# aticejiang/MLAgg-UNet

Hardware: AMD Instinct MI355X
Metric: images/sec (train step) MLAgg-UNet-2D 256x256 bs10 (higher is better)
Workload: dtype f32; 1 GPU; nnUNetTrainer_MLAgg_2D_dt_MS train step, AbdomenMRI-shaped 256x256x1, 14 classes, attention variant B (BASELINE.json configs[1]); batch_per_gpu=10, global_batch=10, parallelism=dp1, launch=eager, miopen=tuned find-db (mlagg-unet_amd/miopen_db), library_gemm=TunableOp table (mlagg-unet_amd/gemm_db), tuning off

## Files before the change

include/mlagg_hip.h:

```cpp
#ifndef MLAGG_HIP_H
#define MLAGG_HIP_H

#include <stddef.h>

#ifdef __cplusplus
extern "C" {
#endif

#define MLAGG_E_UNSUPPORTED (-1)
#define MLAGG_E_NULLPTR     (-2)
#define MLAGG_E_WORKSPACE   (-3)

#define MLAGG_DTYPE_F32  0
#define MLAGG_DTYPE_BF16 1
#define MLAGG_DTYPE_F16  2
#define MLAGG_DTYPE_BF16X3 3

const char *mlagg_version(void);
const char *mlagg_error_string(int code);

int mlagg_profile_kernel_count(void);
const char *mlagg_profile_kernel_name(int id);
int mlagg_profile_select(int id);
int mlagg_profile_collect(double *ms, int *counts);
// ... 55 lines not shown
                              float *dbias, float *workspace, int batch, int H, int W, int C, void *stream);
int mlagg_dwconv3x3_bwd(const float *x, int x_stride, const float *w, const float *dy, int dy_stride,
                        const float *pre, float *dx, int dx_stride, float *dw, float *dbias, float *workspace,
                        int batch, int H, int W, int C, int silu, void *stream);

int mlagg_linear_fwd(const float *x, int x_stride, const float *w, const float *bias, float *y, int y_stride,
                     int M, int N, int K, void *stream);
int mlagg_linear_dgrad(const float *dy, int dy_stride, const float *w, float *dx, int dx_stride, int M, int O, int I,
                       void *stream);
int mlagg_linear_lp_fwd(const float *x, int x_stride, const float *w, const float *bias, float *y, int y_stride,
                        int M, int N, int K, int dtype, void *stream);
int mlagg_linear_lp_dgrad(const float *dy, int dy_stride, const float *w, float *dx, int dx_stride, int M, int O, int I,
                          int dtype, void *stream);
size_t mlagg_linear_wgrad_workspace_floats(int M, int O, int I);
int mlagg_linear_wgrad(const float *dy, int dy_stride, const float *x, int x_stride, float *dW, float *db,
                       float *workspace, int M, int O, int I, void *stream);
int mlagg_linear_wgrad_x3(const float *dy, int dy_stride, const float *x, int x_stride, float *dW, float *db, float *workspace,
                          int M, int O, int I, void *stream);

int mlagg_flash_attn_fwd(const void *q, const void *k, const void *v, void *out, float *lse, int B, int N, int P, int nh,
                         int head_dim, float softmax_scale, int dtype, void *stream);
size_t mlagg_flash_attn_bwd_workspace_floats(int B, int N, int P, int nh, int head_dim);
int mlagg_flash_attn_bwd(const void *q, const void *k, const void *v, const void *out, const void *dout, const float *lse,
                         void *dq, float *workspace, int B, int N, int P, int nh, int head_dim, float softmax_scale,
                         int dtype, void *stream);

int mlagg_layernorm_supported(int C);
int mlagg_layernorm_fwd(const float *x, int x_stride, const float *gamma, const float *beta, float *y,
                        float *stats, int rows, int C, float eps, void *stream);
size_t mlagg_layernorm_bwd_workspace_floats(int rows, int C);
int mlagg_layernorm_bwd(const float *x, int x_stride, const float *dy, int dy_stride, const float *gamma,
                        const float *stats, float *dx, float *dgamma, float *dbeta, float *workspace,
                        int rows, int C, void *stream);
int mlagg_residual_layernorm_fwd(const float *skip, const float *branch, const float *scale, const float *gamma, const float *beta,
                                 float *xsum, float *y, float *stats, int rows, int rows_per_sample, int C, float eps, void *stream);
int mlagg_residual_layernorm_bwd(const float *xsum, const float *dy, int dy_stride, const float *dres, const float *scale,
                                 const float *gamma, const float *stats, float *dskip, float *dbranch, float *dgamma, float *dbeta,
                                 float *workspace, int rows, int rows_per_sample, int C, void *stream);

int mlagg_dwconv3d_fwd(const float *x, int x_stride, const float *w, const float *bias, float *y, int y_stride,
                       float *pre, int batch, int D, int H, int W, int C, int silu, void *stream);
size_t mlagg_dwconv3d_bwd_workspace_floats(int batch, int D, int H, int W, int C);
int mlagg_dwconv3d_bwd(const float *x, int x_stride, const float *w, const float *dy, int dy_stride, const float *pre,
                       float *dx, int dx_stride, float *dw, float *dbias, float *workspace, int batch, int D, int H,
                       int W, int C, int silu, void *stream);

int mlagg_dwconv3x3_nchw_fwd(const float *x, const float *w, const float *bias, float *y, int B, int C, int H, int W,
                             int stride, void *stream);
size_t mlagg_dwconv3x3_nchw_bwd_workspace_floats(int B, int C, int H, int W, int stride);
int mlagg_dwconv3x3_nchw_bwd(const float *x, const float *w, const float *dy, float *dx, float *dw, float *dbias,
                             float *workspace, int B, int C, int H, int W, int stride, void *stream);
int mlagg_dwconv3x3_nchw_bwd_res(const float *x, const float *w, const float *dy, const float *dres, float *dx, float *dw, float *dbias,
                                 float *workspace, int B, int C, int H, int W, int stride, void *stream);

int mlagg_cross_scan(const float *tok, int tok_stride, int blk_stride, float *seq, int B, int nscale,
                     const int *H, const int *W, int CB, int nblk, void *stream);
int mlagg_cross_merge(const float *seq, float *tok, int tok_stride, int blk_stride, int B, int nscale,
                      const int *H, const int *W, int CB, int nblk, void *stream);

int mlagg_conv1x1_supported(int O, int I, long P);
int mlagg_conv1x1_fwd(const float *x, long x_batch, const float *w, const float *bias, float *y, long y_batch, int B, int O, int I,
                      long P, void *stream);
size_t mlagg_conv1x1_wgrad_workspace_floats(int B, int O, int I, long P);
int mlagg_conv1x1_wgrad(const float *dy, long dy_batch, const float *x, long x_batch, float *dW, float *workspace, int B, int O,
                        int I, long P, void *stream);
int mlagg_conv1x1_fwd_lp(const float *x, long x_batch, const float *w, const float *bias, float *y, long y_batch, int B, int O, int I,
                         long P, int dtype, void *stream);
int mlagg_conv1x1_wgrad_lp(const float *dy, long dy_batch, const float *x, long x_batch, float *dW, float *workspace, int B, int O,
                           int I, long P, int dtype, void *stream);
int mlagg_conv1x1_fwd_ragged(const float *x, long x_batch, const float *w, const float *bias, float *y, long y_batch, int B, int O, int I,
                             int I_valid, long P, int dtype, void *stream);
int mlagg_conv1x1_fwd_acc(const float *x, long x_batch, const float *w, const float *bias, float *y, long y_batch, int B, int O, int I,
                          int I_valid, long P, int dtype, int accumulate, void *stream);
int mlagg_conv1x1_fwd_tile(int O);
int mlagg_conv1x1_wgrad_tile(int O, int I);

int mlagg_conv3x3_supported(int O, int I, int H, int W);
size_t mlagg_conv3x3_workspace_bytes(int O, int I);
int mlagg_conv3x3_fwd(const float *x, long x_batch, const float *w, int transposed, const float *bias, float *y, long y_batch,
                      void *workspace, int B, int O, int I, int H, int W, void *stream);
int mlagg_conv3x3x3_supported(int O, int I, int D, int H, int W);
size_t mlagg_conv3x3x3_workspace_bytes(int O, int I);
int mlagg_conv3x3x3_fwd(const float *x, long x_batch, const float *w, int transposed, const float *bias, float *y, long y_batch,
                        void *workspace, int B, int O, int I, int D, int H, int W, void *stream);
int mlagg_conv3x3_wgrad_supported(int O, int I, int H, int W);
int mlagg_conv3x3x3_wgrad_supported(int O, int I, int D, int H, int W);
size_t mlagg_conv3x3x3_wgrad_workspace_floats(int B, int O, int I, int D, int H, int W);
int mlagg_conv3x3x3_wgrad(const float *dy, long dy_batch, const float *x, long x_batch, float *dW, float *workspace, int B, int O,
                          int I, int D, int H, int W, void *stream);
size_t mlagg_conv3x3_wgrad_workspace_floats(int B, int O, int I, int H, int W);
int mlagg_conv3x3_wgrad(const float *dy, long dy_batch, const float *x, long x_batch, float *dW, float *workspace, int B, int O,
                        int I, int H, int W, void *stream);
int mlagg_conv3x3_fwd_lp(const float *x, long x_batch, const float *w, int transposed, const float *bias, float *y, long y_batch,
                         void *workspace, int B, int O, int I, int H, int W, int dtype, void *stream);
int mlagg_conv3x3_wgrad_lp(const float *dy, long dy_batch, const float *x, long x_batch, float *dW, float *workspace, int B, int O,
                           int I, int H, int W, int dtype, void *stream);
int mlagg_conv3x3_fwd_tile(int O, int D, int H, int W);
int mlagg_conv3x3_wgrad_form(int O, int I, int D, int dtype);

int mlagg_conv3x3_s2t_supported(int O, int I, int H, int W);
size_t mlagg_conv3x3_s2t_workspace_bytes(int O, int I);
int mlagg_conv3x3_s2t_fwd(const float *x, long x_batch, const float *w, float *y, long y_batch, void *workspace, int B, int O, int I,
                          int H, int W, int dtype, void *stream);
int mlagg_conv3x3_s2_dgrad(const float *dy, long dy_batch, long dy_chan_stride, long dy_row_stride, const float *w, float *dx,
                           long dx_batch, void *workspace, int B, int O, int I, int H, int W, int dtype, void *stream);
size_t mlagg_conv3x3_s2t_wgrad_workspace_floats(int B, int O, int I, int H, int W);
// ... 242 lines not shown
```

mlagg-unet_amd/csrc/api.hip:

```cpp
#include <hip/hip_runtime.h>

#include <mutex>
#include <vector>

#include "mlagg_hip.h"
#include "prof.h"

namespace mlagg_prof {

int g_selected = -1;

namespace {
struct Rec {
    int id;
    hipEvent_t start, stop;
};
std::mutex g_mu;
std::vector<Rec> g_recs;
size_t g_used = 0;
const char *const kNames[K_COUNT] = {
    "selscan_fwd_kernel<false>", "selscan_chunk_prefix", "selscan_fwd_kernel<true>", "selscan_bwd_local_kernel",
    "selscan_bwd_group_kernel", "selscan_reduce_partials", "local_attn_fwd_kernel", "local_attn_bwd_a_kernel",
    "local_attn_bwd_b_kernel", "pooled_attn_fwd_kernel", "pooled_attn_bwd1_kernel",
    "pooled_attn_bwd2_kernel", "dwconv_tiled_kernel<fwd>", "dwconv_tiled_kernel<dgrad>", "dwconv_bwd_weight_kernel", "linear weight gradient (K5w: linear_wgrad_kernel / linear_wgrad_x3_kernel + reduce)", "layernorm_fwd_kernel",
    "layernorm_bwd_kernel", "dwconv_nchw_fwd_kernel", "dwconv_nchw_bwd (data+weight+reduce)",
    "cross_scan_kernel<false>", "cross_scan_kernel<true>", "gate_fwd_kernel", "gate_bwd_kernel",
    "linear forward + data gradient (K5: linear_x3_kernel on weight images; MLAGG_K5_V2=0: linear_lp_kernel<true, MODE> / linear_mfma_kernel<true>)", "linear data gradient (K5: linear_mfma_kernel<false> / linear_lp_kernel<false, MODE>)", "row_scale_kernel", "dice_ce_stats_kernel", "dice_ce_grad_kernel", "transpose_tile_kernel", "bias gradient (plane_sum / column_sum)", "plane_norm_fwd_kernel", "plane_norm_bwd_kernel", "adamw (sumsq + update)", "flash_fwd_kernel", "flash_bwd (dq + dk/dv)", "channel_epilogue (bias + residual + GELU)",
    "sel1_fwd_kernel<2, false>", "sel1_fwd_kernel<2, true>", "sel1_bwd_local_kernel<2>", "sel1_bwd_kernel<2>",
    "sel1_fwd_kernel<R != 2, false>", "sel1_fwd_kernel<R != 2, true>", "sel1_bwd_local_kernel<R != 2>", "sel1_bwd_kernel<R != 2>",
    "sel1_prefix_kernel", "sel1 reductions (step partials + per-chunk rows)",
    "volume_pad_kernel (+ guard fill)", "conv_wgrad_taps_kernel", "conv_wgrad_reduce_kernel", "conv_taps_kernel (forward / data gradient)",
    "gelu_pool (forward + backward)", "conv1x1 (forward / data gradient / weight gradient)",
    "conv3x3 (forward / data gradient / weight gradient, incl. weight image and reduce)",
    "tok_fwd_kernel<false>", "tok_fwd_kernel<true>", "tok_bwd_local_kernel", "tok_bwd_group_kernel",
    "sw_gather_kernel", "sw_fold_kernel", "sw_finalize_kernel", "resample_linear_kernel", "export_kernel",
    "pp_box_kernel", "pp_stats_kernel (+ final)", "pp_normalize_kernel", "pp_minmax_kernel", "pp_cubic_kernel", "pp_gather_kernel",
    "cc_local_kernel", "cc_merge_kernel", "cc_compress_kernel", "cc_size_kernel", "cc_max_kernel", "cc_write_kernel",
    "sf_stats_kernel (+ init)", "sf_codes_kernel", "sf_zpass_kernel", "sf_ypass_kernel", "sf_xpass_kernel", "sf_sum_kernel",
    "aug3d_resample_kernel", "pt_seg_crop_kernel", "pt_seg_resize_kernel", "pt_rank_count_kernel (+ scan)", "pt_rank_select_kernel",
    "cl_local_kernel", "cl_merge_kernel", "cl_compress_kernel", "cl_flag_kernel", "cl_scan (count + offsets + apply)", "cl_rewrite_kernel",
    "cl_overlap_kernel", "cl_match_kernel", "ens_mean_kernel", "label_confusion_kernel", "dice_bce_stats_kernel", "dice_bce_grad_kernel",
    "aug3d_planar_kernel", "sw_gather_onehot_kernel"};
}

void record(int id, hipStream_t st, bool begin)
{
    std::lock_guard<std::mutex> lk(g_mu);
    if (begin) {
        if (g_used == g_recs.size()) {
            Rec r{id, nullptr, nullptr};
            if (hipEventCreate(&r.start) != hipSuccess || hipEventCreate(&r.stop) != hipSuccess) return;
            g_recs.push_back(r);
        }
        g_recs[g_used].id = id;
        (void)hipEventRecord(g_recs[g_used].start, st);
        ++g_used;
    } else if (g_used > 0) {
        (void)hipEventRecord(g_recs[g_used - 1].stop, st);
    }
}

}

extern "C" const char *mlagg_version(void) { return "mlagg_hip 0.1 (gfx950)"; }

extern "C" const char *mlagg_error_string(int code)
{
    switch (code) {
    case 0: return "success";
    case MLAGG_E_UNSUPPORTED: return "unsupported shape for the gfx950 kernels";
    case MLAGG_E_NULLPTR: return "required pointer argument is NULL";
    case MLAGG_E_WORKSPACE: return "workspace too small";
    default: return code > 0 ? hipGetErrorString(static_cast<hipError_t>(code)) : "unknown mlagg error";
    }
}

extern "C" int mlagg_profile_kernel_count(void) { return mlagg_prof::K_COUNT; }

extern "C" const char *mlagg_profile_kernel_name(int id)
{
    return (id >= 0 && id < mlagg_prof::K_COUNT) ? mlagg_prof::kNames[id] : "?";
}

extern "C" int mlagg_profile_select(int id)
{
    if (id < -2 || id >= mlagg_prof::K_COUNT) return MLAGG_E_UNSUPPORTED;
    mlagg_prof::g_selected = id;
    return 0;
}

extern "C" int mlagg_profile_collect(double *ms, int *counts)
{
    using namespace mlagg_prof;
    if (!ms || !counts) return MLAGG_E_NULLPTR;
    std::lock_guard<std::mutex> lk(g_mu);
// ... 12 lines not shown
```

mlagg-unet_amd/csrc/prof.h:

```cpp
#pragma once
#include <hip/hip_runtime.h>

namespace mlagg_prof {

enum KernelId {
    K_SELSCAN_FWD_LOCAL = 0, K_SELSCAN_PREFIX, K_SELSCAN_FWD_FINAL, K_SELSCAN_BWD_LOCAL, K_SELSCAN_BWD,
    K_SELSCAN_REDUCE, K_LOCAL_FWD, K_LOCAL_BWD_A, K_LOCAL_BWD_B, K_POOLED_FWD,
    K_POOLED_BWD1, K_POOLED_BWD2, K_DWCONV_FWD, K_DWCONV_BWD_DATA, K_DWCONV_BWD_WEIGHT, K_LINEAR_WGRAD, K_LAYERNORM_FWD, K_LAYERNORM_BWD, K_DWCONV_NCHW_FWD, K_DWCONV_NCHW_BWD, K_CROSS_SCAN, K_CROSS_MERGE, K_GATE_FWD, K_GATE_BWD, K_LINEAR_FWD, K_LINEAR_DGRAD, K_ROW_SCALE, K_LOSS_STATS, K_LOSS_GRAD, K_TRANSPOSE, K_BIAS_GRAD, K_PLANE_NORM_FWD, K_PLANE_NORM_BWD, K_ADAMW, K_FLASH_FWD, K_FLASH_BWD, K_CHANNEL_EPI,
    K_SEL1_FWD_LOCAL_R2, K_SEL1_FWD_FINAL_R2, K_SEL1_BWD_LOCAL_R2, K_SEL1_BWD_R2, K_SEL1_FWD_LOCAL, K_SEL1_FWD_FINAL, K_SEL1_BWD_LOCAL,
    K_SEL1_BWD, K_SEL1_PREFIX, K_SEL1_REDUCE, K_CONV_PAD, K_CONV_WGRAD, K_CONV_WGRAD_REDUCE, K_CONV_TAPS, K_GELU_POOL, K_CONV1X1, K_CONV3X3, K_TOK_FWD_LOCAL, K_TOK_FWD_FINAL, K_TOK_BWD_LOCAL, K_TOK_BWD_GROUP, K_SW_GATHER, K_SW_FOLD, K_SW_FINALIZE, K_RESAMPLE_LINEAR, K_EXPORT_SEG, K_PP_BOX, K_PP_STATS, K_PP_NORMALIZE, K_PP_MINMAX, K_PP_CUBIC, K_PP_GATHER, K_CC_LOCAL, K_CC_MERGE, K_CC_COMPRESS, K_CC_SIZE, K_CC_MAX, K_CC_WRITE, K_SF_STATS, K_SF_CODES, K_SF_ZPASS, K_SF_YPASS, K_SF_XPASS, K_SF_SUM, K_AUG3D_RESAMPLE, K_PT_SEG_CROP, K_PT_SEG_RESIZE, K_PT_RANK_COUNTS, K_PT_RANK_SELECT,
    K_CL_LOCAL, K_CL_MERGE, K_CL_COMPRESS, K_CL_FLAG, K_CL_SCAN, K_CL_REWRITE, K_CL_OVERLAP, K_CL_MATCH,
    K_ENS_MEAN, K_LABEL_CONFUSION, K_REGION_LOSS_STATS, K_REGION_LOSS_GRAD, K_AUG3D_PLANAR, K_SW_GATHER_ONEHOT, K_COUNT
};

extern int g_selected;
void record(int id, hipStream_t st, bool begin);

struct Scope {
    int id;
    hipStream_t st;
    bool on;
    Scope(int id_, hipStream_t st_) : id(id_), st(st_), on(g_selected == -2 || g_selected == id_)
    {
        if (on) record(id, st, true);
    }
    ~Scope()
    {
        if (on) record(id, st, false);
    }
};

}

#define MLAGG_TIMED(id, st) mlagg_prof::Scope mlagg_prof_scope_##id(mlagg_prof::id, st)
```

mlagg-unet_amd/model.py:

```python
import math
from typing import Sequence

import torch
import torch.nn as nn
import torch.nn.functional as F

from . import ops

LAMBDA_INIT = 0.8


class _DropPathPool:

    active = None

    def __init__(self):
        self.order, self.keep, self.masks, self.pos, self.recording = [], None, None, 0, False
        self.injected, self.forced = None, False

    def inject(self, factors):
        self.injected = factors

    def begin(self, batch, device):
        if self.injected is not None:
# ... 95 lines not shown
        y = self.raw(x)
        if y.dtype == torch.float32:
            return ops.channel_epilogue(y, self.bias, res if res is None or res.dtype == torch.float32 else res.float(), act)
        if y.numel() // (y.shape[0] * y.shape[1]) % 4:
            return ops.channel_epilogue(y.float(), self.bias, None if res is None else res.float(), act)
        return ops.channel_epilogue_lp(y, self.bias, res, act, dtype or torch.float32)

    def _device_forward(self, x):
        y = self.raw(x)
        if y.dtype == torch.float32:
            return y if self.bias is None else ops.channel_bias(y, self.bias)
        if y.numel() // (y.shape[0] * y.shape[1]) % 4:
            y = y.float()
            return y if self.bias is None else ops.channel_bias(y, self.bias)
        return ops.channel_epilogue_lp(y, self.bias, None, ops.EPI_NONE, torch.float32)


class Conv2d(_ConvMixin, nn.Conv2d):

    def _lib_conv(self, x, w):
        return F.conv2d(x, w, None, self.stride, self.padding, self.dilation, self.groups)

    def _eager(self, x):
        return nn.Conv2d.forward(self, x)

    def forward(self, x):
        if not x.is_cuda or self.padding_mode != "zeros":
            return nn.Conv2d.forward(self, x)
        return self._device_forward(x)


class ConvTranspose2d(_ConvMixin, nn.ConvTranspose2d):
    def _lib_conv(self, x, w):
        return F.conv_transpose2d(x, w, None, self.stride, self.padding, self.output_padding, self.groups, self.dilation)

    def _eager(self, x):
        return nn.ConvTranspose2d.forward(self, x)

    def forward(self, x, output_size=None):
        if not x.is_cuda or output_size is not None:
            return nn.ConvTranspose2d.forward(self, x, output_size)
        return self._device_forward(x)


class GroupNorm(nn.GroupNorm):

    def forward(self, x, out_dtype=None):
        if self.num_groups == self.num_channels and x.is_cuda and x.dim() == 4:
            return ops.plane_norm(x, self.weight, self.bias, self.eps, out_dtype=out_dtype)
        return super().forward(x)


def _chain_dtype(x):
    cdt = ops.conv_dtype()
    pixels = x.numel() // (x.shape[0] * x.shape[1])
    if cdt == torch.float32 or pixels % 4:
        return None
    if pixels >= ops.LP_K_MIN_PIXELS:
        return None
    return cdt


def _instance_norm_act(norm, x, act=ops.ACT_NONE, slope=0.0, res=None, out_dtype=None):
    if x.is_cuda and not norm.track_running_stats:
        return ops.plane_norm(x, norm.weight, norm.bias, norm.eps, act, slope, res, out_dtype or torch.float32)
    y = norm(x) if res is None else norm(x) + res
    return F.leaky_relu(y, slope) if act == ops.ACT_LEAKY else (F.silu(y) if act == ops.ACT_SILU else y)


class Linear(nn.Linear):

    def forward(self, x):
        return ops.linear(x, self.weight, self.bias)


class LayerNorm(nn.LayerNorm):

    def forward(self, x):
        return ops.layer_norm(x, self.weight, self.bias, self.eps)


class Mlp(nn.Module):
    def __init__(self, dim, hidden):
        super().__init__()
        self.fc1 = Linear(dim, hidden)
        self.fc2 = Linear(hidden, dim)

    def forward(self, x):
        return ops.mlp(x, self.fc1.weight, self.fc1.bias, self.fc2.weight, self.fc2.bias)


class RMSNormWeight(nn.Module):

    def __init__(self, dim):
        super().__init__()
        self.weight = nn.Parameter(torch.ones(dim))


class _StackFn(torch.autograd.Function):

    @staticmethod
    def forward(ctx, buf, ranges, *params):
        ctx.ranges, ctx.shapes = ranges, [tuple(p.shape) for p in params]
        return buf.detach()

    @staticmethod
    def backward(ctx, g):
        out, off = [None, None], 0
# ... 245 lines not shown
            for i in range(depth)])

    def forward(self, x):
        B, C, h, w = x.shape
        t = _MapToTokens.apply(x)
        tn = None
        for i, blk in enumerate(self.blocks):
            if i + 1 < len(self.blocks):
                t, tn = blk.forward_tokens(t, tn, self.blocks[i + 1].norm1)
            else:
                t = blk.forward_tokens(t, tn)
        return _TokensToMap.apply(t, h, w)


class Project(nn.Module):
    def __init__(self, cin, cout, stride, last):
        super().__init__()
        self.conv1 = Conv2d(cin, cout, 3, stride=stride, padding=1)
        self.conv2 = Conv2d(cout, cout, 3, stride=1, padding=1)
        self.norm1 = LayerNorm(cout)
        self.last = last
        if not last:
            self.norm2 = LayerNorm(cout)

    @staticmethod
    def _ln(norm, x):
        return _TokensToMap.apply(norm(_MapToTokens.apply(x)), x.shape[2], x.shape[3])

    def forward(self, x):
        x = self._ln(self.norm1, self.conv1.fused(x, act=ops.EPI_GELU))
        return self.conv2(x) if self.last else self._ln(self.norm2, self.conv2.fused(x, act=ops.EPI_GELU))


class PatchEmbed(nn.Module):
    def __init__(self, patch_size, in_chans, embed_dim):
        super().__init__()
        self.proj1 = Project(in_chans, embed_dim // 2, (2, 2), last=False)
        self.proj2 = Project(embed_dim // 2, embed_dim, (patch_size // 2, patch_size // 2), last=True)

    def forward(self, x):
        return self.proj2(self.proj1(x))


class MedNeXtBlock(nn.Module):
    def __init__(self, cin, cout, exp_r, k=3, do_res=True, stride=1):
        super().__init__()
        self.do_res = do_res
        self.conv1 = Conv2d(cin, cin, k, stride=stride, padding=k // 2, groups=cin)
        self.norm = GroupNorm(cin, cin)
        self.conv2 = Conv2d(cin, exp_r * cin, 1)
        self.conv3 = Conv2d(exp_r * cin, cout, 1)

    def body(self, x, res=None):
        pair = ops.dwconv3x3_nchw_res(x, self.conv1.weight, self.conv1.bias) if (res is x and self.conv1.stride[0] == 1) else None
        if pair is not None:
            x1, res = pair
        else:
            x1 = ops.dwconv3x3_nchw(x, self.conv1.weight, self.conv1.bias, self.conv1.stride[0])
        ct = _chain_dtype(x1)
        return self.conv3.fused(self.conv2.fused(self.norm(x1, ct), act=ops.EPI_GELU, dtype=ct), res=res)

    def forward(self, x):
        return self.body(x, x if self.do_res else None)


class MedNeXtDownBlock(MedNeXtBlock):
    def __init__(self, cin, cout, exp_r, k=3):
        super().__init__(cin, cout, exp_r, k, do_res=False, stride=2)
        self.res_conv = Conv2d(cin, cout, 1, stride=2)

    def forward(self, x):
        return self.body(x, self.res_conv.fused(x, dtype=ops.conv_dtype()) if x.is_cuda else self.res_conv(x))


class PatchExpand(nn.Module):
    def __init__(self, cin, cout, k=3):
        super().__init__()
        self.res_conv = ConvTranspose2d(cin, cout, 1, stride=2)
        self.conv1 = ConvTranspose2d(cin, cout, k, stride=2, padding=k // 2)
        self.norm = GroupNorm(cin, cin)

    def forward(self, x):
        ct = _chain_dtype(x)
        res = self.res_conv.fused(x, dtype=ops.conv_dtype()) if x.is_cuda else self.res_conv(x)
        return F.pad(self.conv1.fused(self.norm(x, ct), res=res), (1, 0, 1, 0))


class OutBlock(nn.Module):
    def __init__(self, cin, n_classes):
        super().__init__()
        self.conv_out = ConvTranspose2d(cin, n_classes, 1)

    def forward(self, x):
        return self.conv_out(x)


class _ConvOnly(nn.Module):
    def __init__(self, cin, cout, k, stride=1, transposed=False):
        super().__init__()
        if transposed:
            self.conv = ConvTranspose2d(cin, cout, k, stride=stride, bias=False)
        else:
            self.conv = Conv2d(cin, cout, k, stride=stride, padding=k // 2, bias=False)

    def forward(self, x):
        return self.conv(x)


class UnetResBlock(nn.Module):

    def __init__(self, cin, cout, k=3):
# ... 269 lines not shown
```

mlagg-unet_amd/ops.py:

```python
import ctypes

import numpy as np
import torch

from . import _lib

_launch = _lib.launch
_stream = _lib.stream
_C = _lib.CONSTANTS


PRECISIONS = {"fp32": torch.float32, "bf16": torch.bfloat16, "fp16": torch.float16}
_LP_CODE = {torch.bfloat16: _C["MLAGG_DTYPE_BF16"], torch.float16: _C["MLAGG_DTYPE_F16"]}
import threading as _threading


class _ComputeStack(_threading.local):

    def __init__(self):
        self.stack = [torch.float32]


_COMPUTE = _ComputeStack()

# ... 1760 lines not shown
            inner *= int(v)
        want.reverse()
        plane = inner // int(t.shape[1])
        if tuple(t.stride()[1:]) == tuple(want) and t.stride(0) >= inner and t.stride(0) % plane == 0 and t.stride(0) % 4 == 0 and \
                t.data_ptr() % 16 == 0 and t.dtype in _DT_CODE:
            return t, t.stride(0)
    t = _require_map(t.contiguous(), name)
    return t, 0


class PlaneNormFn(torch.autograd.Function):

    @staticmethod
    def forward(ctx, x, gamma, beta, res, eps, act, slope, out_dtype):
        x = _require_map(x.contiguous(), "x")
        res = None if res is None else _require_map(res.contiguous(), "res", x.shape)
        B, C = x.shape[:2]
        hw = x.numel() // (B * C)
        y = torch.empty(x.shape, device=x.device, dtype=out_dtype or x.dtype)
        stats = torch.empty(B * C, 2, device=x.device, dtype=torch.float32)
        nws = _lib.lib().mlagg_plane_norm_fwd_workspace_floats(B, C, hw)
        ws = torch.empty(nws, device=x.device, dtype=torch.float32) if nws else None
        _launch("mlagg_plane_norm_fwd", _ptr(x), _ptr(gamma), _ptr(beta), _ptr(res), _ptr(y), _ptr(stats), _ptr(ws), B, C, hw, float(eps),
                int(act), float(slope), _DT_CODE[x.dtype], 0 if res is None else _DT_CODE[res.dtype], _DT_CODE[y.dtype])
        ctx.save_for_backward(x, gamma, beta, res, stats)
        ctx.meta = (int(act), float(slope))
        return y

    @staticmethod
    def backward(ctx, dy):
        x, gamma, beta, res, stats = ctx.saved_tensors
        act, slope = ctx.meta
        dy, dyb = _map_slice(dy, "dy")
        B, C = x.shape[:2]
        hw = x.numel() // (B * C)
        lib = _lib.lib()
        dx = torch.empty_like(x)
        dres = torch.empty_like(res) if (res is not None and ctx.needs_input_grad[3]) else None
        dg = torch.empty_like(gamma) if gamma is not None else None
        db = torch.empty_like(beta) if beta is not None else None
        segmented = lib.mlagg_plane_norm_fwd_workspace_floats(B, C, hw) > 0
        ws = torch.empty(lib.mlagg_plane_norm_bwd_workspace_floats(B, C, hw), device=x.device, dtype=torch.float32) \
            if (dg is not None or db is not None or segmented) else None
        _launch("mlagg_plane_norm_bwd_strided", _ptr(x), _ptr(dy), dyb, _ptr(gamma), _ptr(beta), _ptr(res), _ptr(stats), _ptr(dx),
                _ptr(dres), _ptr(dg), _ptr(db), _ptr(ws), B, C, hw, act, slope, _DT_CODE[x.dtype], _DT_CODE[dy.dtype],
                0 if res is None else _DT_CODE[res.dtype])
        return dx, dg, db, dres, None, None, None, None


def plane_norm(x, gamma, beta, eps=1e-5, act=ACT_NONE, slope=0.0, res=None, out_dtype=None):
    return PlaneNormFn.apply(x, gamma, beta, res, eps, act, slope, out_dtype)


class ChannelEpilogueLpFn(torch.autograd.Function):

    @staticmethod
    def forward(ctx, x, bias, res, act, out_dtype):
        x = _require_map(x.contiguous(), "x")
        res = None if res is None else _require_map(res.contiguous(), "res", x.shape)
        B, C = x.shape[:2]
        hw = x.numel() // (B * C)
        y = torch.empty(x.shape, device=x.device, dtype=out_dtype)
        _launch("mlagg_channel_epilogue_lp_fwd", _ptr(x), _DT_CODE[x.dtype], _ptr(bias), _ptr(res),
                0 if res is None else _DT_CODE[res.dtype], _ptr(y), _DT_CODE[y.dtype], B, C, hw, int(act))
        ctx.save_for_backward(x if act == EPI_GELU else None, bias, res if act == EPI_GELU else None)
        ctx.meta = (int(act), x.dtype, None if res is None else res.dtype, tuple(x.shape))
        return y

    @staticmethod
    def backward(ctx, dy):
        x, bias, res = ctx.saved_tensors
        act, xdt, rdt, shape = ctx.meta
        dy = _require_map(dy.contiguous(), "dy", shape)
        B, C = shape[:2]
        hw = dy.numel() // (B * C)
        dx = torch.empty(shape, device=dy.device, dtype=xdt)
        db = torch.empty(C, device=dy.device, dtype=torch.float32) if bias is not None else None
        ws = (torch.empty(_lib.lib().mlagg_channel_sum_workspace_floats(B, C), device=dy.device, dtype=torch.float32)
              if bias is not None else None)
        _launch("mlagg_channel_epilogue_lp_bwd", _ptr(x), _DT_CODE[xdt], _ptr(bias), _ptr(res), 0 if res is None else _DT_CODE[res.dtype],
                _ptr(dy), _DT_CODE[dy.dtype], _ptr(dx), _DT_CODE[xdt], _ptr(db), _ptr(ws), B, C, hw, act)
        dres = None
        if rdt is not None and ctx.needs_input_grad[2]:
            src = dy if act == EPI_NONE else dx
            dres = src if src.dtype == rdt else (dx if dx.dtype == rdt else src.to(rdt))
        return dx, db, dres, None, None


def channel_epilogue_lp(x, bias=None, res=None, act=EPI_NONE, out_dtype=torch.float32):
    return ChannelEpilogueLpFn.apply(x, bias, res, act, out_dtype)


def _planes(t, name):
    _require(t, name)
    inner, want = 1, []
    for v in reversed(t.shape[1:]):
        want.append(inner)
        inner *= int(v)
    want.reverse()
    if tuple(t.stride()[1:]) != tuple(want) or t.stride(0) < inner or t.stride(0) % 4 or t.data_ptr() % 16:
        t = t.contiguous()
    return t, t.stride(0), inner // int(t.shape[1])


K18 = _os.environ.get("MLAGG_K18", "1") == "1"
K18_FWD_MIN_PIXELS = int(_os.environ.get("MLAGG_K18_FWD_MIN_PIXELS", "4096"))
# ... 1305 lines not shown
```

Baseline: 285.1 images/sec.

## Fuse depthwise 3x3 conv with per-channel instance norm in MedNeXt blocks

Adds a HIP kernel pair that computes the depthwise 3x3 convolution and the per-plane GroupNorm (groups == channels) in one pass per plane, keeping the conv output in registers for the statistics. The backward recomputes the conv output instead of storing it, stages the norm gradient in LDS, and produces dx plus the dw, dbias, dgamma and dbeta partials in one kernel, followed by a small reduction kernel. The intent is to remove the intermediate activation's write and read traffic and several separate kernel launches. In exchange the backward does extra conv work, and with up to 1024 threads and a whole plane in LDS per block, occupancy on large planes may be low.

Result: no change. 287.3 images/sec, median of 6 (+0.8%).

```diff
diff --git a/include/mlagg_hip.h b/include/mlagg_hip.h
--- a/include/mlagg_hip.h
+++ b/include/mlagg_hip.h
@@ -131,6 +131,14 @@
                              float *workspace, int B, int C, int H, int W, int stride, void *stream);
 int mlagg_dwconv3x3_nchw_bwd_res(const float *x, const float *w, const float *dy, const float *dres, float *dx, float *dw, float *dbias,
                                  float *workspace, int B, int C, int H, int W, int stride, void *stream);
+
+int mlagg_dwconv_norm_supported(int H, int W, int stride);
+int mlagg_dwconv_norm_fwd(const float *x, const float *w, const float *bias, const float *gamma, const float *beta, float *y,
+                          float *stats, int B, int C, int H, int W, int stride, float eps, void *stream);
+size_t mlagg_dwconv_norm_bwd_workspace_floats(int B, int C);
+int mlagg_dwconv_norm_bwd(const float *x, const float *w, const float *stats, const float *gamma, const float *dy, long dy_batch,
+                          const float *dres, float *dx, float *dw, float *dbias, float *dgamma, float *dbeta, float *workspace,
+                          int B, int C, int H, int W, int stride, void *stream);
 
 int mlagg_cross_scan(const float *tok, int tok_stride, int blk_stride, float *seq, int B, int nscale,
                      const int *H, const int *W, int CB, int nblk, void *stream);
diff --git a/mlagg-unet_amd/csrc/api.hip b/mlagg-unet_amd/csrc/api.hip
--- a/mlagg-unet_amd/csrc/api.hip
+++ b/mlagg-unet_amd/csrc/api.hip
@@ -40,7 +40,7 @@
     "aug3d_resample_kernel", "pt_seg_crop_kernel", "pt_seg_resize_kernel", "pt_rank_count_kernel (+ scan)", "pt_rank_select_kernel",
     "cl_local_kernel", "cl_merge_kernel", "cl_compress_kernel", "cl_flag_kernel", "cl_scan (count + offsets + apply)", "cl_rewrite_kernel",
     "cl_overlap_kernel", "cl_match_kernel", "ens_mean_kernel", "label_confusion_kernel", "dice_bce_stats_kernel", "dice_bce_grad_kernel",
-    "aug3d_planar_kernel", "sw_gather_onehot_kernel"};
+    "aug3d_planar_kernel", "sw_gather_onehot_kernel", "dwconv_norm_fwd_kernel", "dwconv_norm_bwd_kernel"};
 }
 
 void record(int id, hipStream_t st, bool begin)
diff --git a/mlagg-unet_amd/csrc/dwconv_norm.hip b/mlagg-unet_amd/csrc/dwconv_norm.hip
--- /dev/null
+++ b/mlagg-unet_amd/csrc/dwconv_norm.hip
@@ -0,0 +1,413 @@
+#include <hip/hip_runtime.h>
+#include <stdint.h>
+
+#include "mlagg_hip.h"
+#include "prof.h"
+#include "internal.h"
+#include "reduce.h"
+
+namespace {
+
+constexpr int MAX_OUT = 16384;
+constexpr int SMALL_OUT = 4096;
+
+struct DN {
+    int C, H, W, Ho, Wo;
+};
+
+template <int NT>
+__device__ __forceinline__ float block_sum_nt(float v, float *red)
+{
+    v = wave_sum(v);
+    __syncthreads();
+    if ((threadIdx.x & 63) == 0) red[threadIdx.x >> 6] = v;
+    __syncthreads();
+    float s = 0.f;
+#pragma unroll
+    for (int i = 0; i < NT / 64; ++i) s += red[i];
+    return s;
+}
+
+template <int S>
+__device__ __forceinline__ void conv_item(const float *__restrict__ xp, const float (&wk)[9], int H, int W, int oy, int ox0,
+                                          float (&acc)[4 / S], float (&v)[3][6])
+{
+    const int ix0 = ox0 * S;
+    const int cl = max(ix0 - 1, 0), cr = min(ix0 + 4, W - 1);
+    const bool hl = ix0 > 0, hr = ix0 + 4 < W;
+#pragma unroll
+    for (int ky = 0; ky < 3; ++ky) {
+        const int iy = oy * S + ky - 1;
+        const bool ok = iy >= 0 && iy < H;
+        const float *row = xp + (size_t)min(max(iy, 0), H - 1) * W;
+        const float4 m = *reinterpret_cast<const float4 *>(row + ix0);
+        const float l = row[cl];
+        const float r = S == 1 ? row[cr] : 0.f;
+        v[ky][0] = (ok && hl) ? l : 0.f;
+        v[ky][1] = ok ? m.x : 0.f;
+        v[ky][2] = ok ? m.y : 0.f;
+        v[ky][3] = ok ? m.z : 0.f;
+        v[ky][4] = ok ? m.w : 0.f;
+        v[ky][5] = (S == 1 && ok && hr) ? r : 0.f;
+    }
+#pragma unroll
+    for (int ky = 0; ky < 3; ++ky)
+#pragma unroll
+        for (int o = 0; o < 4 / S; ++o)
+            acc[o] += wk[3 * ky] * v[ky][S * o] + wk[3 * ky + 1] * v[ky][S * o + 1] + wk[3 * ky + 2] * v[ky][S * o + 2];
+}
+
+template <int PX>
+__device__ __forceinline__ void load_px(const float *p, float (&d)[PX])
+{
+    if constexpr (PX == 4) {
+        const float4 t = *reinterpret_cast<const float4 *>(p);
+        d[0] = t.x; d[1] = t.y; d[2] = t.z; d[3] = t.w;
+    } else {
+        const float2 t = *reinterpret_cast<const float2 *>(p);
+        d[0] = t.x; d[1] = t.y;
+    }
+}
+
+template <int PX>
+__device__ __forceinline__ void store_px(float *p, const float (&d)[PX])
+{
+    if constexpr (PX == 4) *reinterpret_cast<float4 *>(p) = make_float4(d[0], d[1], d[2], d[3]);
+    else *reinterpret_cast<float2 *>(p) = make_float2(d[0], d[1]);
+}
+
+template <int PX>
+__device__ __forceinline__ float sum_px(const float (&d)[PX])
+{
+    if constexpr (PX == 4) return (d[0] + d[1]) + (d[2] + d[3]);
+    else return d[0] + d[1];
+}
+
+template <int S, int NT>
+__global__ void __launch_bounds__(NT, 4)
+dwconv_norm_fwd_kernel(const float *__restrict__ x, const float *__restrict__ w, const float *__restrict__ bias,
+                       const float *__restrict__ gamma, const float *__restrict__ beta, float *__restrict__ y,
+                       float *__restrict__ stats, DN g, float eps)
+{
+    constexpr int PX = 4 / S, NI = 16 / PX;
+    __shared__ float red[NT / 64];
+    const size_t plane = blockIdx.x;
+    const int c = (int)(plane % g.C);
+    const int WI = g.Wo / PX, nitems = g.Ho * WI;
+    const float HW = (float)(g.Ho * g.Wo);
+    const float *xp = x + plane * g.H * g.W;
+    float *yp = y + plane * g.Ho * g.Wo;
+    float wk[9];
+#pragma unroll
+    for (int j = 0; j < 9; ++j) wk[j] = w[c * 9 + j];
+    const float bv = bias ? bias[c] : 0.f;
+    float x1[NI][PX];
+    float s = 0.f;
+#pragma unroll
+    for (int i = 0; i < NI; ++i) {
+#pragma unroll
+        for (int o = 0; o < PX; ++o) x1[i][o] = 0.f;
+        if (i * NT >= nitems) continue;
+        const int idx = threadIdx.x + i * NT, id = min(idx, nitems - 1);
+        const int oy = id / WI, ox0 = (id - oy * WI) * PX;
+        float acc[PX], v[3][6];
+#pragma unroll
+        for (int o = 0; o < PX; ++o) acc[o] = bv;
+        conv_item<S>(xp, wk, g.H, g.W, oy, ox0, acc, v);
+#pragma unroll
+        for (int o = 0; o < PX; ++o) x1[i][o] = idx < nitems ? acc[o] : 0.f;
+        s += sum_px<PX>(x1[i]);
+    }
+    const float mean = block_sum_nt<NT>(s, red) / HW;
+    float q = 0.f;
+#pragma unroll
+    for (int i = 0; i < NI; ++i) {
+        if (threadIdx.x + i * NT < nitems) {
+#pragma unroll
+            for (int o = 0; o < PX; ++o) x1[i][o] -= mean;
+            float d[PX];
+#pragma unroll
+            for (int o = 0; o < PX; ++o) d[o] = x1[i][o] * x1[i][o];
+            q += sum_px<PX>(d);
+        }
+    }
+    const float rstd = rsqrtf(block_sum_nt<NT>(q, red) / HW + eps);
+    const float ga = gamma[c] * rstd, be = beta[c];
+#pragma unroll
+    for (int i = 0; i < NI; ++i) {
+        const int idx = threadIdx.x + i * NT;
+        if (idx < nitems) {
+            float o4[PX];
+#pragma unroll
+            for (int o = 0; o < PX; ++o) o4[o] = x1[i][o] * ga + be;
+            store_px<PX>(yp + (size_t)idx * PX, o4);
+        }
+    }
+    if (threadIdx.x == 0) { stats[2 * plane] = mean; stats[2 * plane + 1] = rstd; }
+}
+
+template <int S, int NT>
+__global__ void __launch_bounds__(NT, 4)
+dwconv_norm_bwd_kernel(const float *__restrict__ x, const float *__restrict__ w, const float *__restrict__ stats,
+                       const float *__restrict__ gamma, const float *__restrict__ dy, long dy_batch, const float *__restrict__ dres,
+                       float *__restrict__ dx, float *__restrict__ part, DN g)
+{
+    constexpr int PX = 4 / S, NI = 16 / PX, NW = NT / 64;
+    extern __shared__ float4 dwn_lds[];
+    float *pl = reinterpret_cast<float *>(dwn_lds);
+    __shared__ float red[10][NW];
+    const size_t plane = blockIdx.x;
+    const int c = (int)(plane % g.C);
+    const size_t b = plane / g.C;
+    const int Ho = g.Ho, Wo = g.Wo, H = g.H, W = g.W;
+    const int WI = Wo / PX, nitems = Ho * WI;
+    const float HW = (float)(Ho * Wo);
+    const float *xp = x + plane * H * W;
+    const float *gp = dy + b * (size_t)dy_batch + (size_t)c * Ho * Wo;
+    const float *rp = dres ? dres + plane * H * W : nullptr;
+    float *dxp = dx + plane * H * W;
+    float wk[9];
+#pragma unroll
+    for (int j = 0; j < 9; ++j) wk[j] = w[c * 9 + j];
+    const float rstd = stats[2 * plane + 1], k = rstd * gamma[c];
+
+    float xh[NI][PX], gy[NI][PX], xc[NI][4];
+    int pos[NI];
+    float s0 = 0.f;
+#pragma unroll
+    for (int i = 0; i < NI; ++i) {
+        pos[i] = 0;
+#pragma unroll
+        for (int o = 0; o < PX; ++o) { xh[i][o] = 0.f; gy[i][o] = 0.f; }
+#pragma unroll
+        for (int o = 0; o < 4; ++o) xc[i][o] = 0.f;
+        if (i * NT >= nitems) continue;
+        const int idx = threadIdx.x + i * NT, id = min(idx, nitems - 1);
+        const bool live = idx < nitems;
+        const int oy = id / WI, ox0 = (id - oy * WI) * PX;
+        pos[i] = oy << 16 | ox0;
+        float acc[PX], v[3][6], gq[PX];
+#pragma unroll
+        for (int o = 0; o < PX; ++o) acc[o] = 0.f;
+        load_px<PX>(gp + (size_t)id * PX, gq);
+        conv_item<S>(xp, wk, H, W, oy, ox0, acc, v);
+#pragma unroll
+        for (int o = 0; o < PX; ++o) { xh[i][o] = live ? acc[o] : 0.f; gy[i][o] = live ? gq[o] : 0.f; }
+        if (S == 1) {
+#pragma unroll
+            for (int o = 0; o < 4; ++o) xc[i][o] = live ? v[1][o + 1] : 0.f;
+        }
+        s0 += sum_px<PX>(xh[i]);
+    }
+    const float mean = block_sum_nt<NT>(s0, red[0]) / HW;
+    float s1 = 0.f, s2 = 0.f;
+#pragma unroll
+    for (int i = 0; i < NI; ++i) {
+        if (threadIdx.x + i * NT < nitems) {
+            float t[PX];
+#pragma unroll
+            for (int o = 0; o < PX; ++o) { xh[i][o] = (xh[i][o] - mean) * rstd; t[o] = gy[i][o] * xh[i][o]; }
+            s1 += sum_px<PX>(gy[i]);
+            s2 += sum_px<PX>(t);
+        }
+    }
+    const float S1 = block_sum_nt<NT>(s1, red[0]), S2 = block_sum_nt<NT>(s2, red[0]);
+    const float c1 = -k * (S1 / HW), c2 = -k * (S2 / HW);
+
+    float gw[9] = {0.f, 0.f, 0.f, 0.f, 0.f, 0.f, 0.f, 0.f, 0.f};
+    float gb = 0.f;
+#pragma unroll
+    for (int i = 0; i < NI; ++i) {
+        if (i * NT >= nitems) continue;
+        const int idx = threadIdx.x + i * NT;
+        const bool live = idx < nitems;
+        float d1[PX];
+#pragma unroll
+        for (int o = 0; o < PX; ++o) d1[o] = live ? fmaf(c2, xh[i][o], fmaf(k, gy[i][o], c1)) : 0.f;
+        if (S == 2) {
+            float acc[PX], v[3][6];
+#pragma unroll
+            for (int o = 0; o < PX; ++o) acc[o] = 0.f;
+            conv_item<S>(xp, wk, H, W, pos[i] >> 16, pos[i] & 0xffff, acc, v);
+#pragma unroll
+            for (int ky = 0; ky < 3; ++ky)
+#pragma unroll
+                for (int kx = 0; kx < 3; ++kx)
+#pragma unroll
+                    for (int o = 0; o < PX; ++o) gw[3 * ky + kx] += d1[o] * v[ky][S * o + kx];
+            gb += sum_px<PX>(d1);
+        }
+        if (live) store_px<PX>(pl + idx * PX, d1);
+    }
+    __syncthreads();
+
+    if (S == 1) {
+#pragma unroll
+        for (int i = 0; i < NI; ++i) {
+            if (i * NT >= nitems) continue;
+            const int idx = threadIdx.x + i * NT, id = min(idx, nitems - 1);
+            const bool live = idx < nitems;
+            const int oy = pos[i] >> 16, ox0 = pos[i] & 0xffff;
+            float acc[4] = {0.f, 0.f, 0.f, 0.f};
+            if (rp) load_px<4>(rp + (size_t)id * 4, acc);
+            const int cl = max(ox0 - 1, 0), cr = min(ox0 + 4, Wo - 1);
+            const bool hl = ox0 > 0, hr = ox0 + 4 < Wo;
+            float nb[3][6];
+#pragma unroll
+            for (int r = 0; r < 3; ++r) {
+                const int ry = oy + r - 1;
+                const bool ok = live && ry >= 0 && ry < Ho;
+                const float *row = pl + min(max(ry, 0), Ho - 1) * Wo;
+                const float4 m = *reinterpret_cast<const float4 *>(row + ox0);
+                const float l = row[cl], rr = row[cr];
+                nb[r][0] = (ok && hl) ? l : 0.f;
+                nb[r][1] = ok ? m.x : 0.f;
+                nb[r][2] = ok ? m.y : 0.f;
+                nb[r][3] = ok ? m.z : 0.f;
+                nb[r][4] = ok ? m.w : 0.f;
+                nb[r][5] = (ok && hr) ? rr : 0.f;
+            }
+#pragma unroll
+            for (int ky = 0; ky < 3; ++ky)
+#pragma unroll
+                for (int kx = 0; kx < 3; ++kx)
+#pragma unroll
+                    for (int o = 0; o < 4; ++o) {
+                        const float d = nb[2 - ky][o + 2 - kx];
+                        acc[o] += wk[3 * ky + kx] * d;
+                        gw[3 * ky + kx] += xc[i][o] * d;
+                    }
+            gb += (nb[1][1] + nb[1][2]) + (nb[1][3] + nb[1][4]);
+            if (live) store_px<4>(dxp + (size_t)idx * 4, acc);
+        }
+    } else {
+        const int W4 = W >> 2, nin = H * W4;
+        for (int it = threadIdx.x; it < nin; it += NT) {
+            const int iy = it / W4, ix0 = 4 * (it - iy * W4), a = ix0 >> 1;
+            float acc[4] = {0.f, 0.f, 0.f, 0.f};
+            if (rp) load_px<4>(rp + (size_t)it * 4, acc);
+            const int c2 = min(a + 2, Wo - 1);
+            const bool h2 = a + 2 < Wo;
+#pragma unroll
+            for (int ky = 0; ky < 3; ++ky) {
+                const int ty = iy + 1 - ky;
+                const bool ok = ty >= 0 && !(ty & 1) && (ty >> 1) < Ho;
+                const float *row = pl + min(max(ty >> 1, 0), Ho - 1) * Wo;
+                const float2 p = *reinterpret_cast<const float2 *>(row + a);
+                const float t2 = row[c2];
+                const float p0 = ok ? p.x : 0.f, p1 = ok ? p.y : 0.f, p2 = (ok && h2) ? t2 : 0.f;
+                acc[0] += wk[3 * ky + 1] * p0;
+                acc[1] += wk[3 * ky] * p1 + wk[3 * ky + 2] * p0;
+                acc[2] += wk[3 * ky + 1] * p1;
+                acc[3] += wk[3 * ky] * p2 + wk[3 * ky + 2] * p1;
+            }
+            store_px<4>(dxp + (size_t)it * 4, acc);
+        }
+    }
+
+    const int lane = threadIdx.x & 63, wave = threadIdx.x >> 6;
+    __syncthreads();
+#pragma unroll
+    for (int j = 0; j < 10; ++j) {
+        const float t = wave_sum(j < 9 ? gw[j] : gb);
+        if (lane == 0) red[j][wave] = t;
+    }
+    __syncthreads();
+    if (threadIdx.x < 10) {
+        float t = 0.f;
+#pragma unroll
+        for (int i = 0; i < NW; ++i) t += red[threadIdx.x][i];
+        part[plane * 12 + threadIdx.x] = t;
+    }
+    if (threadIdx.x == 0) { part[plane * 12 + 10] = S2; part[plane * 12 + 11] = S1; }
+}
+
+__global__ void __launch_bounds__(256)
+dwconv_norm_finish_kernel(const float *__restrict__ part, int B, int C, float *__restrict__ dw, float *__restrict__ dbias,
+                          float *__restrict__ dgamma, float *__restrict__ dbeta)
+{
+    const int i = blockIdx.x * blockDim.x + threadIdx.x;
+    if (i >= C * 12) return;
+    float s = 0.f;
+    for (int b = 0; b < B; ++b) s += part[(size_t)b * C * 12 + i];
+    const int c = i / 12, j = i - c * 12;
+    if (j < 9) dw[c * 9 + j] = s;
+    else if (j == 9) { if (dbias) dbias[c] = s; }
+    else if (j == 10) dgamma[c] = s;
+    else dbeta[c] = s;
+}
+
+bool make_dn(DN &g, int B, int C, int H, int W, int stride)
+{
+    if (B <= 0 || C <= 0 || (long)B * C > 2147483647L || !mlagg_dwconv_norm_supported(H, W, stride)) return false;
+    g.C = C; g.H = H; g.W = W;
+    g.Ho = (H - 1) / stride + 1;
+    g.Wo = (W - 1) / stride + 1;
+    return true;
+}
+
+inline bool aligned16(const void *p) { return (((uintptr_t)p) & 15) == 0; }
+
+}
+
+extern "C" int mlagg_dwconv_norm_supported(int H, int W, int stride)
+{
+    if (H <= 0 || W <= 0 || (stride != 1 && stride != 2) || (W & 3)) return 0;
+    const long out = (long)((H - 1) / stride + 1) * ((W - 1) / stride + 1);
+    return out <= MAX_OUT ? 1 : 0;
+}
+
+extern "C" int mlagg_dwconv_norm_fwd(const float *x, const float *w, const float *bias, const float *gamma, const float *beta,
+                                     float *y, float *stats, int B, int C, int H, int W, int stride, float eps, void *stream)
+{
+    if (!x || !w || !gamma || !beta || !y || !stats) return MLAGG_E_NULLPTR;
+    DN g;
+    if (!make_dn(g, B, C, H, W, stride) || !aligned16(x) || !aligned16(y)) return MLAGG_E_UNSUPPORTED;
+    hipStream_t st = static_cast<hipStream_t>(stream);
+    MLAGG_TIMED(K_DWCONV_NORM_FWD, st);
+    const bool small = g.Ho * g.Wo <= SMALL_OUT;
+#define MLAGG_DWN_FWD(S, NT) \
+    hipLaunchKernelGGL((dwconv_norm_fwd_kernel<S, NT>), dim3(B * C), dim3(NT), 0, st, x, w, bias, gamma, beta, y, stats, g, eps)
+    if (stride == 1 && small) MLAGG_DWN_FWD(1, 256);
+    else if (stride == 1) MLAGG_DWN_FWD(1, 1024);
+    else if (small) MLAGG_DWN_FWD(2, 256);
+    else MLAGG_DWN_FWD(2, 1024);
+#undef MLAGG_DWN_FWD
+    return (int)hipGetLastError();
+}
+
+extern "C" size_t mlagg_dwconv_norm_bwd_workspace_floats(int B, int C)
+{
+    return (size_t)(B > 0 ? B : 0) * (C > 0 ? C : 0) * 12;
+}
+
+extern "C" int mlagg_dwconv_norm_bwd(const float *x, const float *w, const float *stats, const float *gamma, const float *dy,
+                                     long dy_batch, const float *dres, float *dx, float *dw, float *dbias, float *dgamma,
+                                     float *dbeta, float *workspace, int B, int C, int H, int W, int stride, void *stream)
+{
+    if (!x || !w || !stats || !gamma || !dy || !dx || !dw || !dgamma || !dbeta || !workspace) return MLAGG_E_NULLPTR;
+    DN g;
+    if (!make_dn(g, B, C, H, W, stride)) return MLAGG_E_UNSUPPORTED;
+    const long chw = (long)C * g.Ho * g.Wo;
+    if (dy_batch == 0) dy_batch = chw;
+    if (dy_batch < chw || dy_batch % (4 / stride)) return MLAGG_E_UNSUPPORTED;
+    if (!aligned16(x) || !aligned16(dy) || !aligned16(dx) || (dres && !aligned16(dres))) return MLAGG_E_UNSUPPORTED;
+    hipStream_t st = static_cast<hipStream_t>(stream);
+    MLAGG_TIMED(K_DWCONV_NORM_BWD, st);
+    const bool small = g.Ho * g.Wo <= SMALL_OUT;
+    const size_t lds = (size_t)g.Ho * g.Wo * sizeof(float);
+#define MLAGG_DWN_BWD(S, NT)                                                                                                     \
+    do {                                                                                                                         \
+        if (int rc = mlagg_internal::allow_lds(dwconv_norm_bwd_kernel<S, NT>, lds)) return rc;                                   \
+        hipLaunchKernelGGL((dwconv_norm_bwd_kernel<S, NT>), dim3(B * C), dim3(NT), lds, st, x, w, stats, gamma, dy, dy_batch,    \
+                           dres, dx, workspace, g);                                                                              \
+    } while (0)
+    if (stride == 1 && small) MLAGG_DWN_BWD(1, 256);
+    else if (stride == 1) MLAGG_DWN_BWD(1, 1024);
+    else if (small) MLAGG_DWN_BWD(2, 256);
+    else MLAGG_DWN_BWD(2, 1024);
+#undef MLAGG_DWN_BWD
+    hipLaunchKernelGGL(dwconv_norm_finish_kernel, dim3((C * 12 + 255) / 256), dim3(256), 0, st, workspace, B, C, dw, dbias, dgamma,
+                       dbeta);
+    return (int)hipGetLastError();
+}
diff --git a/mlagg-unet_amd/csrc/prof.h b/mlagg-unet_amd/csrc/prof.h
--- a/mlagg-unet_amd/csrc/prof.h
+++ b/mlagg-unet_amd/csrc/prof.h
@@ -10,7 +10,7 @@
     K_SEL1_FWD_LOCAL_R2, K_SEL1_FWD_FINAL_R2, K_SEL1_BWD_LOCAL_R2, K_SEL1_BWD_R2, K_SEL1_FWD_LOCAL, K_SEL1_FWD_FINAL, K_SEL1_BWD_LOCAL,
     K_SEL1_BWD, K_SEL1_PREFIX, K_SEL1_REDUCE, K_CONV_PAD, K_CONV_WGRAD, K_CONV_WGRAD_REDUCE, K_CONV_TAPS, K_GELU_POOL, K_CONV1X1, K_CONV3X3, K_TOK_FWD_LOCAL, K_TOK_FWD_FINAL, K_TOK_BWD_LOCAL, K_TOK_BWD_GROUP, K_SW_GATHER, K_SW_FOLD, K_SW_FINALIZE, K_RESAMPLE_LINEAR, K_EXPORT_SEG, K_PP_BOX, K_PP_STATS, K_PP_NORMALIZE, K_PP_MINMAX, K_PP_CUBIC, K_PP_GATHER, K_CC_LOCAL, K_CC_MERGE, K_CC_COMPRESS, K_CC_SIZE, K_CC_MAX, K_CC_WRITE, K_SF_STATS, K_SF_CODES, K_SF_ZPASS, K_SF_YPASS, K_SF_XPASS, K_SF_SUM, K_AUG3D_RESAMPLE, K_PT_SEG_CROP, K_PT_SEG_RESIZE, K_PT_RANK_COUNTS, K_PT_RANK_SELECT,
     K_CL_LOCAL, K_CL_MERGE, K_CL_COMPRESS, K_CL_FLAG, K_CL_SCAN, K_CL_REWRITE, K_CL_OVERLAP, K_CL_MATCH,
-    K_ENS_MEAN, K_LABEL_CONFUSION, K_REGION_LOSS_STATS, K_REGION_LOSS_GRAD, K_AUG3D_PLANAR, K_SW_GATHER_ONEHOT, K_COUNT
+    K_ENS_MEAN, K_LABEL_CONFUSION, K_REGION_LOSS_STATS, K_REGION_LOSS_GRAD, K_AUG3D_PLANAR, K_SW_GATHER_ONEHOT, K_DWCONV_NORM_FWD, K_DWCONV_NORM_BWD, K_COUNT
 };
 
 extern int g_selected;
diff --git a/mlagg-unet_amd/model.py b/mlagg-unet_amd/model.py
--- a/mlagg-unet_amd/model.py
+++ b/mlagg-unet_amd/model.py
@@ -171,8 +171,11 @@
 
 
 def _chain_dtype(x):
+    return _chain_dtype_of(x.numel() // (x.shape[0] * x.shape[1]))
+
+
+def _chain_dtype_of(pixels):
     cdt = ops.conv_dtype()
-    pixels = x.numel() // (x.shape[0] * x.shape[1])
     if cdt == torch.float32 or pixels % 4:
         return None
     if pixels >= ops.LP_K_MIN_PIXELS:
@@ -524,11 +527,21 @@
         self.conv3 = Conv2d(exp_r * cin, cout, 1)
 
     def body(self, x, res=None):
-        pair = ops.dwconv3x3_nchw_res(x, self.conv1.weight, self.conv1.bias) if (res is x and self.conv1.stride[0] == 1) else None
+        stride = self.conv1.stride[0]
+        Ho, Wo = (x.shape[2] - 1) // stride + 1, (x.shape[3] - 1) // stride + 1
+        if x.is_cuda and _chain_dtype_of(Ho * Wo) is None and self.norm.num_groups == self.norm.num_channels:
+            with_res = res is x and stride == 1 and ops.DWC_RES and x.requires_grad and torch.is_grad_enabled()
+            xn = ops.dwconv3x3_norm_nchw(x, self.conv1.weight, self.conv1.bias, self.norm.weight, self.norm.bias, self.norm.eps, stride,
+                                         with_res)
+            if xn is not None:
+                if with_res:
+                    xn, res = xn
+                return self.conv3.fused(self.conv2.fused(xn, act=ops.EPI_GELU, dtype=None), res=res)
+        pair = ops.dwconv3x3_nchw_res(x, self.conv1.weight, self.conv1.bias) if (res is x and stride == 1) else None
         if pair is not None:
             x1, res = pair
         else:
-            x1 = ops.dwconv3x3_nchw(x, self.conv1.weight, self.conv1.bias, self.conv1.stride[0])
+            x1 = ops.dwconv3x3_nchw(x, self.conv1.weight, self.conv1.bias, stride)
         ct = _chain_dtype(x1)
         return self.conv3.fused(self.conv2.fused(self.norm(x1, ct), act=ops.EPI_GELU, dtype=ct), res=res)
 
diff --git a/mlagg-unet_amd/ops.py b/mlagg-unet_amd/ops.py
--- a/mlagg-unet_amd/ops.py
+++ b/mlagg-unet_amd/ops.py
@@ -1836,6 +1836,66 @@
     return PlaneNormFn.apply(x, gamma, beta, res, eps, act, slope, out_dtype)
 
 
+DWNORM = int(_os.environ.get("MLAGG_DWNORM", "1"))
+
+
+class DWConvNormNCHWFn(torch.autograd.Function):
+
+    @staticmethod
+    def forward(ctx, x, weight, bias, gamma, beta, eps, stride, with_res):
+        x = _require(x.contiguous(), "x")
+        B, C, H, W = x.shape
+        w = _require(weight.reshape(C, 9).contiguous(), "weight")
+        gamma, beta = _require(gamma.contiguous(), "gamma", (C,)), _require(beta.contiguous(), "beta", (C,))
+        Ho, Wo = (H - 1) // stride + 1, (W - 1) // stride + 1
+        y = torch.empty(B, C, Ho, Wo, device=x.device, dtype=torch.float32)
+        stats = torch.empty(B * C, 2, device=x.device, dtype=torch.float32)
+        _launch("mlagg_dwconv_norm_fwd", _ptr(x), _ptr(w), _ptr(bias), _ptr(gamma), _ptr(beta), _ptr(y), _ptr(stats), B, C, H, W,
+                int(stride), float(eps))
+        ctx.save_for_backward(x, w, gamma, stats)
+        ctx.meta = (int(stride), bias is not None, weight.shape)
+        ctx.set_materialize_grads(False)
+        return (y, x.view_as(x)) if with_res else y
+
+    @staticmethod
+    def backward(ctx, dy, dres=None):
+        x, w, gamma, stats = ctx.saved_tensors
+        stride, has_bias, wshape = ctx.meta
+        B, C, H, W = x.shape
+        if dy is None:
+            return dres, None, None, None, None, None, None, None
+        dy, dyb = _map_slice(dy, "dy")
+        if dy.dtype != torch.float32:
+            dy, dyb = dy.float().contiguous(), 0
+        if dres is not None:
+            dres = _require_map(dres.contiguous(), "dres", x.shape)
+            if dres.dtype != torch.float32:
+                dres = dres.float()
+        dx = torch.empty_like(x)
+        dw = torch.empty(C, 9, device=x.device, dtype=torch.float32)
+        db = torch.empty(C, device=x.device, dtype=torch.float32) if has_bias else None
+        dg, dbeta = torch.empty_like(gamma), torch.empty_like(gamma)
+        ws = torch.empty(_lib.lib().mlagg_dwconv_norm_bwd_workspace_floats(B, C), device=x.device, dtype=torch.float32)
+        _launch("mlagg_dwconv_norm_bwd", _ptr(x), _ptr(w), _ptr(stats), _ptr(gamma), _ptr(dy), dyb, _ptr(dres), _ptr(dx), _ptr(dw),
+                _ptr(db), _ptr(dg), _ptr(dbeta), _ptr(ws), B, C, H, W, stride)
+        return dx, dw.reshape(wshape), db, dg, dbeta, None, None, None
+
+
+def dwconv_norm_applies(x, weight, gamma, beta, stride):
+    if DWNORM < int(stride) or gamma is None or beta is None:
+        return False
+    if not (isinstance(x, torch.Tensor) and x.is_cuda and x.dim() == 4 and x.dtype == torch.float32 and weight.dtype == torch.float32
+            and tuple(weight.shape[1:]) == (1, 3, 3)):
+        return False
+    return bool(_lib.lib().mlagg_dwconv_norm_supported(int(x.shape[2]), int(x.shape[3]), int(stride)))
+
+
+def dwconv3x3_norm_nchw(x, weight, bias, gamma, beta, eps=1e-5, stride=1, with_res=False):
+    if not dwconv_norm_applies(x, weight, gamma, beta, stride):
+        return None
+    return DWConvNormNCHWFn.apply(x, weight, bias, gamma, beta, eps, stride, bool(with_res))
+
+
 class ChannelEpilogueLpFn(torch.autograd.Function):
 
     @staticmethod
```
